# WeijingShi/Point-GNN

Measured on AMD Instinct MI355X. Metric: KITTI-shaped frames/sec (car_auto_T3 inference: graph build + GNN, 20000 pts/frame, mean E1 602k), higher is better.
Workload: dtype f32

## Files before the change

include/pointgnn_hip.h:

```cpp
#ifndef POINTGNN_HIP_H_
#define POINTGNN_HIP_H_

#include <stddef.h>
#include <stdint.h>

#ifdef __cplusplus
extern "C" {
#endif

#define PGNN_E_INVALID (-1)
#define PGNN_E_WORKSPACE (-2)
#define PGNN_E_UNSUPPORTED (-3)
#define PGNN_E_CAPACITY (-4)
#define PGNN_E_COMM (-5)

int pgnn_version(void);
const char *pgnn_last_error(void);
int pgnn_check_device_pointer(const void *device_ptr);

int pgnn_stream_create_cu_mask(int32_t cu_first, int32_t cu_count,
                               int32_t complement, void **stream_out);
int pgnn_stream_destroy(void *stream);

int pgnn_scatter_max_f32(const float *data, int64_t ld_data,
// ... 304 lines not shown
    int32_t edges_sorted, float *out, int64_t ld_out, int32_t *sched_ws,
    int32_t aggregation, void *workspace, size_t workspace_bytes, void *stream);
int pgnn_point_set_pooling_agg_fwd_dyn(
    const float *point_features, int32_t n_feat, const float *point_xyz,
    const int32_t *keypoint_indices, const int32_t *edges, int64_t edges_cap,
    int32_t keypoints_cap, const pgnn_fc_layer *layers_host, int32_t n_layers,
    int32_t edges_sorted, float *out, int64_t ld_out, int32_t *sched_ws,
    const pgnn_dyn_count *n_edges, const pgnn_dyn_count *num_keypoints,
    int32_t aggregation, void *workspace, size_t workspace_bytes, void *stream);

size_t pgnn_packed_fc_bf16x3_bytes(int32_t k_in, int32_t n_out);
int pgnn_pack_fc_bf16x3(const float *w_host, const float *b_host, int32_t k_in,
                        int32_t n_out, void *image_host);
int pgnn_edge_mlp_scatter_max_bf16x3_fwd(
    const float *P, const float *Q, int64_t ld_pq, int32_t width,
    const int32_t *edges, int64_t edges_cap, int32_t vertices_cap,
    const void *image, int32_t n_out, int32_t relu_from, int32_t edges_sorted,
    float *out, int64_t ld_out, const pgnn_dyn_count *n_edges,
    const pgnn_dyn_count *num_vertices, void *stream);

size_t pgnn_packed_fc_f16x2_bytes(int32_t k_in, int32_t n_out);
int pgnn_pack_fc_f16x2(const float *w_host, const float *b_host, int32_t k_in,
                       int32_t n_out, void *image_host);
int pgnn_edge_mlp_scatter_max_f16x2_fwd(
    const float *P, const float *Q, int64_t ld_pq, int32_t width,
    const int32_t *edges, int64_t edges_cap, int32_t vertices_cap,
    const void *image, int32_t n_out, int32_t relu_from, int32_t edges_sorted,
    float *out, int64_t ld_out, int32_t *status, const pgnn_dyn_count *n_edges,
    const pgnn_dyn_count *num_vertices, void *stream);

int pgnn_edge_ws_applies(const pgnn_fc_layer *layers_host, int32_t n_layers,
                         int32_t width, int64_t edges_expected, void *stream,
                         int32_t *applies);
int pgnn_edge_mlp_scatter_max_scaled_fwd(
    const float *P, const float *Q, int64_t ld_pq, int32_t width,
    const int32_t *edges, int64_t edges_cap, int32_t vertices_cap,
    const pgnn_fc_layer *layers_host, int32_t n_layers, int32_t edges_sorted,
    float *out, int64_t ld_out, int32_t *sched_ws, int32_t scale_exp,
    int32_t *status, const pgnn_dyn_count *n_edges,
    const pgnn_dyn_count *num_vertices, void *stream);
int pgnn_debug_pk_sub_clamp(const float *a, const float *b, float *out,
                            int32_t n_pairs, void *stream);

int pgnn_pack_fc_f16x2_acc(const float *w_host, const float *b_host,
                           int32_t k_in, int32_t n_out, void *image_host);
int pgnn_point_set_pooling_f16x2_fwd(
    const float *point_features, int32_t n_feat, const float *point_xyz,
    const int32_t *keypoint_indices, const int32_t *edges, int64_t edges_cap,
    int32_t keypoints_cap, const pgnn_fc_layer *layers, int32_t n_layers,
    const void *last_image, const void *hidden_image, int32_t edges_sorted,
    float *out, int64_t ld_out, int32_t *sched_ws, int32_t *status,
    const pgnn_dyn_count *n_edges, const pgnn_dyn_count *num_keypoints,
    void *stream);

int pgnn_edge_mlp_scatter_max_rows_fwd(const float *P, const float *Q,
                                       int64_t ld_pq, int32_t width,
                                       const int32_t *edges, int64_t n_edges,
                                       int32_t num_vertices,
                                       const pgnn_fc_layer *layer_host,
                                       int32_t edges_sorted, float *out,
                                       int64_t ld_out, float *rows_out,
                                       int64_t ld_rows, float *h1_out,
                                       void *stream);

int pgnn_offset_apply(const float *xyz, const float *delta, int64_t ld_delta,
                      int64_t n_rows, const float *wx, float *xyz_out,
// ... 607 lines not shown
```

point-gnn_amd/_lib.py:

```python
import ctypes
import os

import torch

from . import _header

_HERE = os.path.dirname(os.path.abspath(__file__))
LIB_PATH = os.environ.get("PGNN_LIB") or os.path.join(_HERE, "libpointgnn_hip.so")

c_i32, c_i64, c_vp = ctypes.c_int32, ctypes.c_int64, ctypes.c_void_p

_S, _C = _header.structs(), _header.constants()

FcLayer = _S["pgnn_fc_layer"]
DynCount = _S["pgnn_dyn_count"]
WgradJob = _S["pgnn_wgrad_job"]
MergeJob = _S["pgnn_merge_job"]
FrameArrays = _S["pgnn_frame_arrays"]
TrainFc = _S["pgnn_train_fc"]
TrainStage = _S["pgnn_train_stage"]
TrainModel = _S["pgnn_train_model"]
TrainBatch = _S["pgnn_train_batch"]


class PackJob(ctypes.Structure):
    _fields_ = [("w", c_vp), ("b", c_vp), ("dst", c_vp), ("k_in", c_i32),
                ("n_out", c_i32), ("kind", c_i32), ("first_block", c_i32),
                ("ld", c_i32), ("reserved", c_i32)]


PGNN_MAX_LAYERS = _C["PGNN_MAX_LAYERS"]
MERGE_MAX_LEVELS = _C["PGNN_MERGE_MAX_LEVELS"]
TRAIN_MAX_FC = _C["PGNN_TRAIN_MAX_FC"]
TRAIN_MAX_STAGES = _C["PGNN_TRAIN_MAX_STAGES"]
TRAIN_MAX_CLASSES = _C["PGNN_TRAIN_MAX_CLASSES"]
TRAIN_MAX_LEVELS = _C["PGNN_TRAIN_MAX_LEVELS"]
E_INVALID = _C["PGNN_E_INVALID"]
E_WORKSPACE = _C["PGNN_E_WORKSPACE"]
E_UNSUPPORTED = _C["PGNN_E_UNSUPPORTED"]
AGG_MAX, AGG_SUM, AGG_MEAN = (_C["PGNN_AGG_MAX"], _C["PGNN_AGG_SUM"],
                              _C["PGNN_AGG_MEAN"])
SCHED_WS_INTS = _C["PGNN_SCHED_WS_INTS"]


class PointGnnHipError(RuntimeError):
    pass


_lib = None


def exported_symbols():
    return sorted(_header.functions())


def _build_missing():
    import fcntl
    import shutil
    if not (shutil.which("hipcc") or os.path.exists("/opt/rocm/bin/hipcc")):
        return
    lock = os.path.join(os.path.dirname(LIB_PATH), ".build.lock")
    with open(lock, "w") as f:
        fcntl.flock(f, fcntl.LOCK_EX)
        try:
            if not os.path.exists(LIB_PATH):
                from . import build as _build
                _build.build(verbose=False)
        finally:
            fcntl.flock(f, fcntl.LOCK_UN)


def load():
    global _lib
    if _lib is not None:
        return _lib
# ... 87 lines not shown
```

point-gnn_amd/csrc/core.hip:

```cpp
#include <cmath>
#include <string.h>

#include <mutex>
#include <vector>

#include "pgnn_common.h"

namespace pgnn {

std::string &last_error() {
  static thread_local std::string err;
  return err;
}

namespace {
__global__ void sched_zero_kernel(int32_t *sched) {
  if (threadIdx.x < PGNN_SCHED_WS_INTS) sched[threadIdx.x] = 0;
}
}

int arm_sched(int32_t *sched, hipStream_t stream) {
  if (!sched) return 0;
  static_assert(PGNN_SCHED_WS_INTS <= 64, "one wave zeroes the counters");
  hipLaunchKernelGGL(sched_zero_kernel, dim3(1), dim3(64), 0, stream, sched);
// ... 371 lines not shown

extern "C" size_t pgnn_packed_fc_bf16x3_bytes(int32_t k_in, int32_t n_out) {
  return packed_split_bytes<SplitBf16x3>(k_in, n_out);
}

extern "C" size_t pgnn_packed_fc_f16x2_bytes(int32_t k_in, int32_t n_out) {
  return packed_split_bytes<SplitF16x2>(k_in, n_out);
}

extern "C" int pgnn_pack_fc_bf16x3(const float *w, const float *b, int32_t k_in,
                                   int32_t n_out, void *image) {
  PGNN_GUARD_BEGIN
  PGNN_REQUIRE(w && image && k_in > 0 && n_out > 0, PGNN_E_INVALID,
               "pack_fc_bf16x3: bad argument");
  pack_fc_split<SplitBf16x3>(w, b, k_in, n_out, image, false);
  return 0;
  PGNN_GUARD_END
}

extern "C" int pgnn_pack_fc_f16x2(const float *w, const float *b, int32_t k_in,
                                  int32_t n_out, void *image) {
  PGNN_GUARD_BEGIN
  return pack_fc_f16x2(w, b, k_in, n_out, image, false);
  PGNN_GUARD_END
}

extern "C" int pgnn_pack_fc_f16x2_acc(const float *w, const float *b,
                                      int32_t k_in, int32_t n_out, void *image) {
  PGNN_GUARD_BEGIN
  return pack_fc_f16x2(w, b, k_in, n_out, image, true);
  PGNN_GUARD_END
}

extern "C" int pgnn_pack_fc(const float *w, const float *b, int32_t k_in,
                            int32_t n_out, float *packed) {
  PGNN_GUARD_BEGIN
  PGNN_REQUIRE(w && packed && k_in > 0 && n_out > 0, PGNN_E_INVALID,
               "pack_fc: bad argument");
  const int kq = (k_in + 15) / 16, nt = (n_out + 15) / 16;
  for (int q = 0; q < kq; ++q)
    for (int t = 0; t < nt; ++t)
      for (int lane = 0; lane < 64; ++lane)
        for (int s = 0; s < 4; ++s) {
          const int k = 16 * q + 4 * (lane >> 4) + s;
          const int n = 16 * t + (lane & 15);
          packed[(((size_t)q * nt + t) * 64 + lane) * 4 + s] =
              (k < k_in && n < n_out) ? w[(size_t)k * n_out + n] : 0.0f;
        }
  float *bias = packed + (size_t)kq * nt * 256;
  for (int n = 0; n < nt * 16; ++n) bias[n] = (b && n < n_out) ? b[n] : 0.0f;
  return 0;
  PGNN_GUARD_END
}
```

point-gnn_amd/csrc/edge_ws.h:

```cpp
#pragma once
#include "mlp_engine.h"
#include "ws_partition.h"

namespace pgnn {

#ifndef PGNN_WS_SCHED
#define PGNN_WS_SCHED 2
#endif

constexpr int kWsWaves = 8;
constexpr int kWsSchedInts = 2 + kWsMaxSlices * kWsMaxGroups;
constexpr int kWsStampTiles = 38;
constexpr int kWsStampStride = 8 + 4 * kWsStampTiles;

struct EdgeWsArgs {
  const float *P, *Q;
  int ldv4;
  const int32_t *edges;
  int64_t n_edges;
  const int32_t *n_dev;
  const float *wp;
  int nt;
  int relu_from;
  float *out;
// ... 147 lines not shown
  }
  while (pos < 16) {
    if (cur_has)
      ws_flush<NTG, ARGS, SCALED>(a, bias_lds, t0, lane, cur_d, carry,
                    a.sorted && cur_left_closed &&
                        (!fin || d_after != cur_d),
                    inf);
    if (fin) break;
    const unsigned rest = starts & ~((2u << pos) - 1u);
    const int nextpos = rest ? __builtin_ctz(rest) : 16;
    const bool in_run = n >= pos && n < nextpos;
#pragma unroll
    for (int t = 0; t < NTG; ++t)
#pragma unroll
      for (int r = 0; r < 4; ++r)
        carry[t][r] = in_run ? acc[t][r] : kFloatLowest;
    cur_d = __builtin_amdgcn_readlane(my_d, pos);
    cur_left_closed = true;
    cur_has = true;
    pos = nextpos;
  }
  st.cur_d = cur_d;
  st.left_closed = cur_left_closed;
  st.has = cur_has;
}

}

#include "ws_sum.h"

namespace pgnn {

template <int KQ, int NTG, bool EMIT, bool ROWS = false, class POL = WsMax,
          bool SCALED = false>
__device__ __forceinline__ void edge_ws_body(const EdgeWsArgs &a,
                                             const v4f *__restrict__ wl, int t0,
                                             const float *bias_lds,
                                             int64_t tile_first,
                                             int64_t tile_last, int lane,
                                             long long *tsw, int &stamped,
                                             const int64_t E) {
  static_assert(!SCALED || (!EMIT && !ROWS && !POL::kSum),
                "the scaled form exists for the plain max kernel only");
  if (tile_first >= tile_last) return;
  const int n = lane & 15;
  const int64_t e_first = tile_first * 16;
  const int64_t e_end = tile_last * 16 < E ? tile_last * 16 : E;
  const v4f *__restrict__ P4 = reinterpret_cast<const v4f *>(a.P);
  const v4f *__restrict__ Q4 = reinterpret_cast<const v4f *>(a.Q);
  const int2 *__restrict__ e2 = reinterpret_cast<const int2 *>(a.edges);

  int cur_d = e_first > 0 ? a.edges[2 * (e_first - 1) + 1] : -1;
  int d_after = e_end < E ? a.edges[2 * e_end + 1] : -1;
  cur_d = __builtin_amdgcn_readfirstlane(cur_d);
  d_after = __builtin_amdgcn_readfirstlane(d_after);
  bool cur_left_closed = false, cur_has = false;
  constexpr float kIdentity = POL::kSum ? 0.0f : kFloatLowest;
  v4f carry[NTG];
#pragma unroll
  for (int t = 0; t < NTG; ++t)
    carry[t] = (v4f){kIdentity, kIdentity, kIdentity, kIdentity};

  const float inf = opaque_inf();
  bool nxt_ok = e_first + n < E;
  int2 nxt = e2[nxt_ok ? e_first + n : 0];
  for (int64_t tile = tile_first;; ++tile) {
    const bool fin = tile >= tile_last;
    const int64_t e0 = tile * 16;
    if (a.prio) __builtin_amdgcn_s_setprio(3);
    int lz;
    asm volatile("v_mov_b32 %0, %1" : "=v"(lz) : "v"(lane));
    const int g = lz >> 4;
    int lz1 = lz + 64 * 64, lz2 = lz + 128 * 64;
    asm volatile("" : "+v"(lz1));
    asm volatile("" : "+v"(lz2));
    const v4f *__restrict__ wfrag[3] = {wl + lz, wl + lz1, wl + lz2};
// ... 64 lines not shown
        for (int q = 0; q < KQ; ++q) hrow[4 * q] = in[q];
      }
    }
    __builtin_amdgcn_sched_barrier(0);
    if (tst) {
      const long long c = __builtin_readcyclecounter();
      if (lane == 0) tst[1] = c;
      __builtin_amdgcn_sched_barrier(0);
    }
    __builtin_amdgcn_s_setprio(0);
    {
      v4f w[2][NTG];
#pragma unroll
      for (int t = 0; t < NTG; ++t) {
        acc[t] = (v4f){0.f, 0.f, 0.f, 0.f};
        w[0][t] = wfrag[0][t * 64];
      }
      __builtin_amdgcn_sched_barrier(0);
#pragma unroll
      for (int q = 0; q < KQ; ++q) {
        __builtin_amdgcn_s_waitcnt(0xC07F);
        __builtin_amdgcn_sched_barrier(0);
        if (q + 1 < KQ) {
#pragma unroll
          for (int t = 0; t < NTG; ++t)
#ifdef PGNN_WS_ABL_NO_LDS
            w[(q + 1) & 1][t] = w[q & 1][t];
#else
            w[(q + 1) & 1][t] = wfrag[((q + 1) * NTG + t) >> 6]
                                     [(((q + 1) * NTG + t) & 63) * 64];
#endif
        }
#pragma unroll
        for (int s = 0; s < 4; ++s)
#pragma unroll
          for (int t = 0; t < NTG; ++t)
            acc[t] = __builtin_amdgcn_mfma_f32_16x16x4f32(
                w[q & 1][t][s], in[q][s], acc[t], 0, 0, 0);
#if PGNN_WS_SCHED == 2
#pragma unroll
        for (int t = 0; t < NTG; ++t) {
          __builtin_amdgcn_sched_group_barrier(0x8 , 3, 0);
          if (q + 1 < KQ)
            __builtin_amdgcn_sched_group_barrier(0x100 , 1, 0);
        }
        __builtin_amdgcn_sched_group_barrier(0x8 , NTG, 0);
#else
        if (q + 1 < KQ)
          __builtin_amdgcn_sched_group_barrier(0x100 , NTG, 0);
        __builtin_amdgcn_sched_group_barrier(0x8 , 4 * NTG, 0);
#endif
        __builtin_amdgcn_sched_barrier(0);
      }
    }
    if (tst) {
      const long long c = __builtin_readcyclecounter();
      if (lane == 0) tst[2] = c;
      __builtin_amdgcn_sched_barrier(0);
    }
    if constexpr (EMIT) {
      const int64_t row = e0 + n;
      if (row < E) {
        float *dstp = a.rows_out + row * a.ld_rows + 16 * t0 + 4 * g;
#pragma unroll
        for (int t = 0; t < NTG; ++t) {
          const v4f bb = *reinterpret_cast<const v4f *>(bias_lds + 16 * t + 4 * g);
          v4f y;
#pragma unroll
          for (int r = 0; r < 4; ++r) {
            float x = acc[t][r] + bb[r];
            if (16 * (t0 + t) + 4 * g + r >= a.relu_from) x = x > 0.0f ? x : 0.0f;
            y[r] = x;
          }
          *reinterpret_cast<v4f *>(dstp + 16 * t) = y;
        }
      }
    }
    if (a.prio) __builtin_amdgcn_s_setprio(3);
    const int up = __shfl_up(my_d, 1);
// ... 134 lines not shown
                         __HIP_MEMORY_SCOPE_AGENT);
    }
  }
}

__device__ __forceinline__ void ws_scaled_guard(const EdgeWsArgs &a) {
  if (!a.status) return;
  int nv = a.num_segments;
  if (a.nv_dev) {
    const int d = *a.nv_dev;
    nv = d < nv ? d : nv;
  }
  const v4f *__restrict__ P4 = reinterpret_cast<const v4f *>(a.P);
  const v4f *__restrict__ Q4 = reinterpret_cast<const v4f *>(a.Q);
  float m = 0.0f;
  bool bad = false;
  const int mine = nv > (int)blockIdx.x
                       ? (nv - (int)blockIdx.x + (int)gridDim.x - 1) / (int)gridDim.x
                       : 0;
  for (int it = threadIdx.x; it < mine * a.ldv4; it += 64 * kWsWaves) {
    const int j = it / a.ldv4, c = it - j * a.ldv4;
    const size_t at = ((size_t)blockIdx.x + (size_t)j * gridDim.x) * a.ldv4 + c;
    const v4f p = P4[at], q = Q4[at];
#pragma unroll
    for (int i = 0; i < 4; ++i) {
      m = fmaxf(m, fmaxf(fabsf(p[i]), fabsf(q[i])));
      bad |= !(p[i] == p[i]) || !(q[i] == q[i]);
    }
  }
  if (bad || !(m <= 0.5f)) atomicOr(a.status, 1);
}

template <int KQ, int NTMAX, bool EMIT = false, bool ROWS = false,
          class POL = WsMax, bool SCALED = false>
__global__ __launch_bounds__(64 * kWsWaves) void edge_ws_kernel(EdgeWsArgs a) {
  extern __shared__ __attribute__((aligned(16))) char smem[];
  v4f *wl = reinterpret_cast<v4f *>(smem);
  float *bias_lds = reinterpret_cast<float *>(wl + KQ * NTMAX * 64);
  const int lane = threadIdx.x & 63;
  const int wave = __builtin_amdgcn_readfirstlane(threadIdx.x >> 6);
  const int slice = blockIdx.x % a.xcds;
  const int local = blockIdx.x / a.xcds;
  if constexpr (SCALED) ws_scaled_guard(a);
  const long long rt_entry = a.ts ? (long long)__builtin_amdgcn_s_memrealtime() : 0;
  const int grp = ws_group(a, slice, local, wave);
  const int t0 = a.tile0[grp];
  const int ntg = a.tile0[grp + 1] - t0;
  {
    const v4f *__restrict__ src = reinterpret_cast<const v4f *>(a.wp);
    constexpr int PER = (KQ * NTMAX + kWsWaves - 1) / kWsWaves;
    const int n_frag = KQ * ntg;
    v4f tmp[PER];
#pragma unroll
    for (int i = 0; i < PER; ++i) {
      const int f = wave + i * kWsWaves;
      const int fc = f < n_frag ? f : 0;
      const int q = fc / ntg, t = fc - q * ntg;
      tmp[i] = src[((size_t)q * a.nt + t0 + t) * 64 + lane];
    }
    __builtin_amdgcn_sched_barrier(0);
#pragma unroll
    for (int i = 0; i < PER; ++i) {
      const int f = wave + i * kWsWaves;
      if (f < n_frag) wl[(size_t)f * 64 + lane] = tmp[i];
    }
    if ((int)threadIdx.x < 16 * ntg)
      bias_lds[threadIdx.x] =
          a.wp[(size_t)KQ * a.nt * 256 + 16 * t0 + threadIdx.x];
  }
  __syncthreads();
  const int64_t n_edges = ws_edge_count(a.n_edges, a.n_dev);
  const WsShare s = ws_share(a, grp, slice, local, wave, (n_edges + 15) / 16);
  int64_t span = s.last - s.first;
  const int64_t pool = ws_pool_size(span, a.sched, a.pool_pct, 4, s.nw);
  span -= pool;
  const int64_t pool_first = s.first + span;
  int64_t tile_first = s.first + span * s.wi / s.nw;
  int64_t tile_last = s.first + span * (s.wi + 1) / s.nw;
  long long *tsw = nullptr;
  if (a.ts) {
    tsw = a.ts + ((int64_t)blockIdx.x * kWsWaves + wave) * kWsStampStride;
    if (lane == 0) {
      tsw[0] = __builtin_readcyclecounter();
      tsw[2] = __builtin_amdgcn_s_memrealtime();
      tsw[4] = tile_last - tile_first;
      tsw[5] = ntg + 100 * slice;
      tsw[6] = rt_entry;
    }
  }
  int stamped = 0;
  int32_t *counter = a.sched ? a.sched + 2 + slice * kWsMaxGroups + grp : nullptr;
  for (;;) {
    if (ntg == NTMAX)
      edge_ws_body<KQ, NTMAX, EMIT, ROWS, POL, SCALED>(
          a, wl, t0, bias_lds, tile_first, tile_last, lane, tsw, stamped,
          n_edges);
    else
      edge_ws_body<KQ, NTMAX - 1, EMIT, ROWS, POL, SCALED>(
          a, wl, t0, bias_lds, tile_first, tile_last, lane, tsw, stamped,
          n_edges);
    if (pool == 0) break;
    const int c = ws_pool_claim(counter, a.chunk, lane);
    if (c >= pool) break;
    tile_first = pool_first + c;
    tile_last = tile_first + a.chunk < s.last ? tile_first + a.chunk : s.last;
  }
  if (tsw && lane == 0) {
    tsw[1] = __builtin_readcyclecounter();
    tsw[3] = __builtin_amdgcn_s_memrealtime();
    tsw[7] = stamped;
  }
  if (a.sched && lane == 0) {
    const int total = (int)gridDim.x * kWsWaves;
    const int done = __hip_atomic_fetch_add(&a.sched[1], 1, __ATOMIC_ACQ_REL,
                                            __HIP_MEMORY_SCOPE_AGENT);
    if (done == total - 1) {
      for (int i = 0; i < a.xcds * kWsMaxGroups; ++i)
        __hip_atomic_store(&a.sched[2 + i], 0, __ATOMIC_RELAXED,
                           __HIP_MEMORY_SCOPE_AGENT);
      __hip_atomic_store(&a.sched[1], 0, __ATOMIC_RELEASE,
                         __HIP_MEMORY_SCOPE_AGENT);
    }
  }
}

}
```

point-gnn_amd/csrc/gnn.hip:

```cpp
#include <atomic>

#include "mlp_engine.h"
#include "edge_ws.h"
#include "edge_ws_split.h"
#include "pool_ws.h"
#include "pool_split.h"
#include "pool_ws_f16.h"

namespace pgnn {
int g_mlp_blocks_per_cu = 4;
int g_edge_msub = 0;
int g_pool_msub = 0;
int g_mlp_pool_pct = 12;
int g_ws_xcds = 8;
int g_ws_prio = 1;
int g_f16_pool = 1;
int g_b16_force = 0;
int g_ws_pool_pct = 0;
int g_ws_chunk = 2;
int g_ws_balance = 1;
int g_ws_reserve = 0;
void *g_mlp_ts = nullptr;
int g_mlp_debug = 0;
}
// ... 1170 lines not shown
  Plan p;
  const int rc = make_plan(layers, n_layers, width, p);
  if (rc) return rc;
  *applies = edge_ws_applies(p, edges_expected, ws_cus((hipStream_t)stream_));
  return 0;
  PGNN_GUARD_END
}

extern "C" int pgnn_edge_mlp_scatter_max_scaled_fwd(
    const float *P, const float *Q, int64_t ld_pq, int32_t width,
    const int32_t *edges, int64_t edges_cap, int32_t vertices_cap,
    const pgnn_fc_layer *layers, int32_t n_layers, int32_t edges_sorted,
    float *out, int64_t ld_out, int32_t *sched_ws, int32_t scale_exp,
    int32_t *status, const pgnn_dyn_count *n_edges,
    const pgnn_dyn_count *num_vertices, void *stream_) {
  PGNN_GUARD_BEGIN
  hipStream_t stream = (hipStream_t)stream_;
  PGNN_REQUIRE(edges_cap >= 0 && vertices_cap >= 0 && width > 0,
               PGNN_E_INVALID, "edge_mlp_scaled: bad sizes");
  PGNN_REQUIRE(scale_exp >= 0 && scale_exp <= 24, PGNN_E_INVALID,
               "edge_mlp_scaled: scale_exp outside 0..24");
  PGNN_REQUIRE((n_edges == nullptr) == (num_vertices == nullptr) &&
                   (!n_edges || (n_edges->dev && num_vertices->dev)),
               PGNN_E_INVALID, "edge_mlp_scaled: counts come as a pair");
  const Dyn de = dyn_of(n_edges), dk = dyn_of(num_vertices);
  Plan p;
  int rc = make_plan(layers, n_layers, width, p);
  if (rc) return rc;
  PGNN_REQUIRE(ld_pq == 16 * p.chain.l[0].kq, PGNN_E_INVALID,
               "edge_mlp_scaled: ld_pq must equal the padded width 16*ceil(width/16)");
  PGNN_REQUIRE(ld_out >= 16 * p.chain.l[n_layers - 1].nt, PGNN_E_INVALID,
               "edge_mlp_scaled: ld_out < padded output width");
  const int cus = ws_cus(stream);
  if (edges_cap == 0 || vertices_cap == 0 ||
      !edge_ws_applies(p, expected(de, edges_cap), cus))
    return PGNN_E_UNSUPPORTED;
  PGNN_REQUIRE(out && P && Q && edges, PGNN_E_INVALID,
               "edge_mlp_scaled: null pointer");
  PGNN_REQUIRE(((uintptr_t)P % 16 == 0) && ((uintptr_t)Q % 16 == 0),
               PGNN_E_INVALID, "edge_mlp_scaled: P/Q must be 16-byte aligned");
  if (!(edges_sorted & 2)) {
    rc = fill_lowest_rows(out, ld_out, vertices_cap, dk, stream);
    if (rc) return rc;
  }
  const EdgeArgs ea = {P, Q, ld_pq, edges};
  const SegArgs sa = {out, ld_out, vertices_cap, edges_sorted & 1};
  if (p.chain.l[0].nt == 19)
    return launch_edge_ws_scaled<19, 7>(p.chain.l[0], ea, edges_cap, sa, cus,
                                        sched_ws, stream, de.dev, dk.dev,
                                        scale_exp, status);
  return launch_edge_ws_scaled<16, 8>(p.chain.l[0], ea, edges_cap, sa, cus,
                                      sched_ws, stream, de.dev, dk.dev,
                                      scale_exp, status);
  PGNN_GUARD_END
}

extern "C" int pgnn_edge_mlp_scatter_max_bf16x3_fwd(
    const float *P, const float *Q, int64_t ld_pq, int32_t width,
    const int32_t *edges, int64_t edges_cap, int32_t vertices_cap,
    const void *image, int32_t n_out, int32_t relu_from, int32_t edges_sorted,
    float *out, int64_t ld_out, const pgnn_dyn_count *n_edges,
    const pgnn_dyn_count *num_vertices, void *stream_) {
  PGNN_GUARD_BEGIN
  return edge_split_fwd_impl<Bf16x3>(P, Q, ld_pq, width, edges, edges_cap,
                                     vertices_cap, image, n_out, relu_from,
                                     edges_sorted, out, ld_out, nullptr, n_edges,
                                     num_vertices, (hipStream_t)stream_);
  PGNN_GUARD_END
}

extern "C" int pgnn_edge_mlp_scatter_max_f16x2_fwd(
    const float *P, const float *Q, int64_t ld_pq, int32_t width,
    const int32_t *edges, int64_t edges_cap, int32_t vertices_cap,
    const void *image, int32_t n_out, int32_t relu_from, int32_t edges_sorted,
    float *out, int64_t ld_out, int32_t *status, const pgnn_dyn_count *n_edges,
    const pgnn_dyn_count *num_vertices, void *stream_) {
  PGNN_GUARD_BEGIN
  return edge_split_fwd_impl<F16x2>(P, Q, ld_pq, width, edges, edges_cap,
                                    vertices_cap, image, n_out, relu_from,
// ... 1230 lines not shown
```

point-gnn_amd/csrc/ws_launch.h:

```cpp
#pragma once
#include "ws_partition.h"

namespace {
using namespace pgnn;

inline int ws_cus(int cus) {
  return (g_ws_reserve > 0 && cus - g_ws_reserve >= 64) ? cus - g_ws_reserve : cus;
}
inline int ws_cus(hipStream_t stream) { return ws_cus(stream_cu_count(stream)); }

inline int ws_slices(int cus) { return ws_slice_count(cus, g_ws_xcds); }
inline bool ws_feasible(int nt, int ntmax, int cus) {
  return pgnn::ws_feasible(nt, ntmax, cus, ws_slices(cus));
}

inline int ws_partition_rc(int why) {
  PGNN_REQUIRE(why != kWsTooFewCus, PGNN_E_UNSUPPORTED,
               "edge_ws: too few CUs for the column groups");
  PGNN_REQUIRE(why == kWsOk, PGNN_E_UNSUPPORTED,
               "edge_ws: column tiles do not group");
  return 0;
}

template <int KQ, int NTMAX>
// ... 4 lines not shown
  a = {};
  const int rc = ws_partition_rc(ws_partition(a, L.nt, NTMAX, cus, ws_slices(cus)));
  if (rc) return rc;
  a.n_dev = n_dev;
  a.rows_out = rows_out;
  a.ld_rows = ld_rows;
  a.h1_out = h1_out;
  a.P = ea.P;
  a.Q = ea.Q;
  a.ldv4 = (int)(ea.ldpq >> 2);
  a.edges = ea.edges;
  a.n_edges = n_edges;
  a.wp = L.wp;
  a.nt = L.nt;
  a.relu_from = L.relu_from;
  a.out = sa.out;
  a.ldo = sa.ldo;
  a.num_segments = sa.num_segments;
  a.sorted = sa.sorted;
  a.prio = g_ws_prio;
  a.ts = (long long *)g_mlp_ts;
  a.sched = (g_ws_pool_pct > 0 && a.xcds <= kWsMaxSlices) ? sched : nullptr;
  a.pool_pct = g_ws_pool_pct;
  a.chunk = g_ws_chunk;
  if (g_ws_balance >= 2) {
    double cost[kWsMaxGroups];
    for (int g = 0; g < a.groups; ++g)
      cost[g] = 128.0 * KQ * (a.tile0[g + 1] - a.tile0[g]) + 1900.0;
    ws_balance(a, cus, cost, a.sched != nullptr);
  }
  return 0;
}

template <int KQ, int NTMAX, bool ROWS, class POL = WsMax, bool SCALED = false>
int run_edge_ws(const EdgeWsArgs &a, int cus, hipStream_t stream) {
  static_assert(!POL::kSum || !ROWS, "the sum kernels read no ready rows");
  static_assert(!SCALED || (!POL::kSum && !ROWS), "scaled: the plain max kernel only");
  PGNN_HIP((hipError_t)arm_sched(a.sched, stream));
  const size_t lds = (size_t)KQ * NTMAX * 1024 + 16 * NTMAX * sizeof(float);
  auto kern = edge_ws_kernel<KQ, NTMAX, false, ROWS, POL, SCALED>;
  if constexpr (!ROWS && !POL::kSum && !SCALED) {
    if (a.rows_out) kern = edge_ws_kernel<KQ, NTMAX, true>;
  }
  return launch_lds(kern, dim3((unsigned)(cus / a.xcds * a.xcds)),
                    dim3(64 * kWsWaves), lds, stream, a);
}

template <int KQ, int NTMAX, class POL = WsMax>
int launch_edge_ws(const LayerDev &L, const EdgeArgs &ea, int64_t n_edges,
                   const SegArgs &sa, int cus, int32_t *sched,
                   hipStream_t stream, float *rows_out = nullptr,
                   int64_t ld_rows = 0, float *h1_out = nullptr,
                   const int32_t *n_dev = nullptr) {
  EdgeWsArgs a;
  const int rc = plan_edge_ws<KQ, NTMAX>(a, L, ea, n_edges, sa, cus, sched,
                                         rows_out, ld_rows, h1_out, n_dev);
  return rc ? rc : run_edge_ws<KQ, NTMAX, false, POL>(a, cus, stream);
}

template <int KQ, int NTMAX>
int launch_edge_ws_scaled(const LayerDev &L, const EdgeArgs &ea, int64_t n_edges,
                          const SegArgs &sa, int cus, int32_t *sched,
                          hipStream_t stream, const int32_t *n_dev,
                          const int32_t *nv_dev, int scale_exp, int32_t *status) {
  EdgeWsArgs a;
  const int rc = plan_edge_ws<KQ, NTMAX>(a, L, ea, n_edges, sa, cus, sched,
                                         nullptr, 0, nullptr, n_dev);
  if (rc) return rc;
  a.nv_dev = nv_dev;
  a.unscale = (float)((int64_t)1 << scale_exp);
  a.status = status;
  return run_edge_ws<KQ, NTMAX, false, WsMax, true>(a, cus, stream);
}

template <class POL = WsMax>
bool edge_ws_applies(const Plan &p, int64_t n_edges, int cus) {
  if (g_mlp_debug & 2048) return false;
  const LayerDev &L = p.chain.l[0];
  if (p.chain.n != 1 || L.kq != L.nt || (L.nt != 19 && L.nt != 16)) return false;
  if (cus < 64 || cus % 8 != 0) return false;
  if (!ws_feasible(L.nt, L.nt == 19 ? 7 : 8, cus)) return false;
  if ((size_t)L.kq * (L.nt == 19 ? 7 : 8) * 1024 + 16 * 8 * sizeof(float) >
      device_max_lds())
    return false;
  if (g_mlp_debug & 4096) return true;
  return n_edges >= (int64_t)16 * 2 * kWsWaves * cus;
}

template <class POL = WsMax>
bool pool_ws_applies(const Plan &p, int64_t n_edges, int cus) {
  if (g_mlp_debug & (8192 | 1024)) return false;
  const ChainDev &c = p.chain;
  if (c.n != 4 || c.l[0].kq != 1 || c.l[0].nt != 2 || c.l[1].nt != 4 ||
      c.l[2].nt != 8 || c.l[3].kq != 8 || c.l[3].nt != 19)
    return false;
  if (cus < 8) return false;
  if ((size_t)8 * 19 * 1024 + 16 * 19 * sizeof(float) > device_max_lds())
    return false;
  if (g_mlp_debug & 16384) return true;
  return n_edges >= (int64_t)16 * 2 * kWsWaves * cus;
}

PoolWsArgs pool_ws_args(const Plan &p, const PoolArgs &pa, int64_t n_edges,
                        const int32_t *n_dev, int num_segments) {
  PoolWsArgs a = {};
  a.feat = pa.feat;
  a.nfeat = pa.nfeat;
  a.xyz = pa.xyz;
  a.kp = pa.kp;
  a.edges = pa.edges;
  a.n_edges = n_edges;
  a.n_dev = n_dev;
  a.l0 = p.chain.l[0];
  a.l1 = p.chain.l[1];
  a.l2 = p.chain.l[2];
  a.wp = p.chain.l[3].wp;
  a.kq = p.chain.l[3].kq;
  a.nt = p.chain.l[3].nt;
  a.relu_from = p.chain.l[3].relu_from;
// ... 183 lines not shown
```

point-gnn_amd/gnn.py:

```python
import contextlib
import ctypes
import threading
from functools import partial

import numpy as np
import torch

from . import _lib
from .weights import mlp_names

__all__ = ["PointSetPooling", "GraphNetAutoCenter", "ClassAwarePredictor",
           "fuse_vertex_stages",
           "multi_layer_neural_network_fn", "multi_layer_fc_fn",
           "graph_scatter_max_fn", "graph_scatter_sum_fn",
           "graph_scatter_mean_fn", "ParamStore", "parameters",
           "variable_scope", "padded_width"]


def padded_width(n):
    return (int(n) + 15) // 16 * 16


class ParamStore(object):

    def __init__(self, params, device=None):
        self.params = {k: np.asarray(v) for k, v in params.items()}
        self.device = device
        self._cache = {}
        self._edge_arith = 'f32'
        self.edge_scaled = False
        self.inference = True

    @property
    def edge_arith(self):
        return self._edge_arith

    @edge_arith.setter
    def edge_arith(self, value):
        if value not in EDGE_ARITHS:
            raise ValueError("edge_arith must be one of %r, not %r"
                             % (EDGE_ARITHS, value))
        self._edge_arith = value

    def range_status(self):
        if getattr(self, '_range_status', None) is None:
            self._range_status = torch.zeros(1, dtype=torch.int32,
                                             device=self._dev())
        return self._range_status

    def edge_range_ok(self):
        st = getattr(self, '_range_status', None)
        if st is None:
            return True
        ok = int(st.item()) == 0
        if not ok:
            st.zero_()
        return ok

    def edge_scale_exp(self, scope):
        scales = self.__dict__.setdefault('_edge_scale', {})
        pend = self.__dict__.setdefault('_edge_scale_pending', {})
        if scope not in scales and scope in pend and \
                not torch.cuda.is_current_stream_capturing():
# ... 66 lines not shown
    def _dev(self):
        if self.device is None:
            if not torch.cuda.is_available():
                raise _lib.PointGnnHipError(
                    "pointgnn_amd needs a GPU: there is no CPU fallback")
            self.device = torch.device("cuda", torch.cuda.current_device())
        return self.device

    def has(self, name):
        return name + '/weights' in self.params

    def fc(self, name):
        w = self.params[name + '/weights']
        if name + '/biases' in self.params:
            return (w.astype(np.float32),
                    self.params[name + '/biases'].astype(np.float32))
        bn = name + '/BatchNorm/'
        if bn + 'moving_mean' not in self.params:
            raise KeyError("%s: neither biases nor BatchNorm statistics"
                           % name)
        mean = self.params[bn + 'moving_mean'].astype(np.float64)
        var = self.params[bn + 'moving_variance'].astype(np.float64)
        s = 1.0 / np.sqrt(var + BATCH_NORM_EPSILON)
        if bn + 'gamma' in self.params:
            s = s * self.params[bn + 'gamma'].astype(np.float64)
        beta = self.params[bn + 'beta'].astype(np.float64) \
            if bn + 'beta' in self.params else 0.0
        return ((w.astype(np.float64) * s).astype(np.float32),
                (beta - mean * s).astype(np.float32))

    def mlp(self, scope, n_layers):
        return [self.fc(n) for n in mlp_names(scope, n_layers)]

    def pack(self, w, b):
        lib = _lib.load()
        w = np.ascontiguousarray(w, dtype=np.float32)
        b = np.ascontiguousarray(b, dtype=np.float32)
        k_in, n_out = w.shape
        host = np.empty(lib.pgnn_packed_fc_floats(k_in, n_out), np.float32)
        _lib.check(lib.pgnn_pack_fc(w.ctypes.data, b.ctypes.data, k_in, n_out,
                                    host.ctypes.data), "pgnn_pack_fc")
        return torch.from_numpy(host).to(self._dev())

    def cached(self, key, builder):
        if key not in self._cache:
            self._cache[key] = builder()
        return self._cache[key]

    def invalidate(self):
        self._cache.clear()


class Chain(object):

    def __init__(self, store, layers):
        self.buffers = []
        self.array = (_lib.FcLayer * len(layers))()
        self.n = len(layers)
        for i, (w, b, relu_from) in enumerate(layers):
            buf = store.pack(w, b)
            self.buffers.append(buf)
            self.array[i].packed = buf.data_ptr()
            self.array[i].k_in = int(w.shape[0])
            self.array[i].n_out = int(w.shape[1])
            self.array[i].relu_from = int(relu_from)
        self.k_in = int(layers[0][0].shape[0])
        self.n_out = int(layers[-1][0].shape[1])


class _State(threading.local):

    def __init__(self):
        self.store = None
        self.scope = []
        self.fuse = False
        self.pending = None
        self.taken = None


_state = _State()


@contextlib.contextmanager
def parameters(store):
    prev = _state.store
    _state.store = store
    try:
        yield store
    finally:
        _state.store = prev


@contextlib.contextmanager
# ... 403 lines not shown
                "pgnn_point_set_pooling_workspace_bytes")
        if done:
            pass
        elif ws_bytes.value:
            work = torch.empty(ws_bytes.value // 4, dtype=torch.float32,
                               device=xyz.device)
            _lib.check(lib.pgnn_point_set_pooling_fwd_ws(
                *args, cnt_e.arg() if cnt_e is not None else None,
                cnt_k.arg() if cnt_k is not None else None, _lib.ptr(work),
                ws_bytes.value, _lib.stream_ptr()),
                "pgnn_point_set_pooling_fwd_ws")
        elif cnt_k is None and cnt_e is None:
            _lib.check(lib.pgnn_point_set_pooling_fwd(
                *args, _lib.stream_ptr()), "pgnn_point_set_pooling_fwd")
        else:
            _lib.check(lib.pgnn_point_set_pooling_fwd_dyn(
                *args, cnt_e.arg(), cnt_k.arg(), _lib.stream_ptr()),
                "pgnn_point_set_pooling_fwd_dyn")
        if AGGREGATE_TAP is not None:
            AGGREGATE_TAP.append(agg)
        with variable_scope('combined_features'):
            out_chain = _relu_chain(store, _scope(),
                                    list(output_MLP_depth_list), False)
        return _finish_rows(out_chain, agg, point_chain.n_out, count=cnt_k)


EDGE_INPUT_TAP = None

EDGE_ARITHS = ('f32', 'bf16x3', 'f16x2')

EDGE_SCALE_HEADROOM = 0.125
EDGE_SCALE_ROWS, EDGE_SCALE_SLOTS = 64, 16


def edge_scale_exp_for(max_abs):
    k = 0
    while k < 24 and not max_abs * 2.0 ** -k <= EDGE_SCALE_HEADROOM:
        k += 1
    return k


class GraphNetAutoCenter(object):

    def __init__(self, edge_feature_fn=multi_layer_neural_network_fn,
                 aggregation_fn=graph_scatter_max_fn,
                 update_fn=multi_layer_neural_network_fn,
                 auto_offset_fn=multi_layer_neural_network_fn):
        self._aggregation = _aggregation_code(aggregation_fn)
        self._edge_feature_fn = edge_feature_fn
        self._aggregation_fn = aggregation_fn
        self._update_fn = update_fn
        self._auto_offset_fn = auto_offset_fn

    def apply_regular(self, input_vertex_features, input_vertex_coordinates,
                      NOT_USED, edges, edge_MLP_depth_list=None,
                      edge_MLP_normalization_type='fused_BN_center',
                      edge_MLP_activation_type='ReLU',
                      update_MLP_depth_list=None,
                      update_MLP_normalization_type='fused_BN_center',
                      update_MLP_activation_type='ReLU', auto_offset=False,
                      auto_offset_MLP_depth_list=None,
                      auto_offset_MLP_normalization_type='fused_BN_center',
                      auto_offset_MLP_feature_activation_type='ReLU'):
        _check_kinds(edge_MLP_activation_type, edge_MLP_normalization_type)
        _check_kinds(update_MLP_activation_type, update_MLP_normalization_type)
        pend = _take_pending(input_vertex_features)
# ... 20 lines not shown
            fcs = store.mlp(edge_scope, len(edge_widths))
            w1, b1 = fcs[0]
            c = w1.shape[0] - 3
            p_chain = Chain(store, [(w1, b1, w1.shape[1])])
            wq = padded_width(w1.shape[1])
            wx = np.zeros((3, wq), np.float32)
            wx[:, :w1.shape[1]] = w1[c:c + 3]
            wx_dev = torch.from_numpy(wx).to(store._dev())
            if len(fcs) > 1:
                rest = Chain(store, [(w, b, 0) for (w, b) in fcs[1:]])
            else:
                rest = None
            return c, p_chain, wx_dev, rest
        c, p_chain, wx_dev, rest = store.cached(
            ('edge', edge_scope, tuple(edge_widths)), build_edge)
        if rest is None:
            raise NotImplementedError("edge MLP needs at least two layers")
        assert h.shape[1] >= c, "vertex features narrower than edge MLP input"

        scale_k, calibrate = None, False
        if store.edge_scaled and store.inference and rest.n == 1 and \
                store.edge_arith == 'f32' and \
                self._aggregation == _lib.AGG_MAX:
            n_exp = int(e.shape[0])
            if cnt_e is not None and 0 < cnt_e.hint < n_exp:
                n_exp = cnt_e.hint
            applies = ctypes.c_int32(0)
            _lib.check(lib.pgnn_edge_ws_applies(
                rest.array, rest.n, int(rest.k_in), n_exp, st,
                ctypes.byref(applies)), "pgnn_edge_ws_applies")
            if applies.value:
                scale_k = store.edge_scale_exp(edge_scope)
                calibrate = scale_k is None and cnt_k is None
        if scale_k is not None:
            def build_scaled():
                w1, b1 = store.mlp(edge_scope, len(edge_widths))[0]
                s = np.float32(2.0 ** -scale_k)
                wx = np.zeros((3, padded_width(w1.shape[1])), np.float32)
                wx[:, :w1.shape[1]] = w1[c:c + 3] * s
                made = (Chain(store, [(w1 * s, b1 * s, w1.shape[1])]),
                        torch.from_numpy(wx).to(store._dev()))
                torch.cuda.current_stream().synchronize()
                return made
            p_chain, wx_dev = store.cached(
                ('edge_scaled', edge_scope, tuple(edge_widths), scale_k),
                build_scaled)

        off_chain = None
        if auto_offset:
            _check_kinds(auto_offset_MLP_feature_activation_type,
                         auto_offset_MLP_normalization_type)
            off_chain = _relu_chain(store, scope,
                                    list(auto_offset_MLP_depth_list), True)
            assert off_chain.k_in == c, "offset MLP input must be the features"
        wq = int(wx_dev.shape[1])
        q = torch.empty((k, wq), dtype=torch.float32, device=h.device)
        p = torch.empty((k, wq), dtype=torch.float32, device=h.device)
        agg = torch.empty((k, padded_width(rest.n_out)), dtype=torch.float32,
                          device=h.device)
        pre_args = (_lib.ptr(h), h.stride(0), c, _lib.ptr(x),
                    off_chain.array if off_chain is not None else None,
                    off_chain.n if off_chain is not None else 0, p_chain.array,
                    _lib.ptr(wx_dev), k, _lib.ptr(p), _lib.ptr(q), wq,
                    _lib.ptr(agg), agg.stride(0))
        if pend is not None:
            res = pend.residual
            front = (_lib.ptr(pend.x), pend.x.stride(0), pend.nx,
                     pend.chain.array, pend.chain.n, _lib.ptr(res),
                     res.stride(0) if res is not None else 0, _lib.ptr(h),
                     h.stride(0))
            if cnt_k is None:
                rc = lib.pgnn_vertex_update_pre_edge_fwd(
                    *(front + pre_args[2:]), st)
            else:
                rc = lib.pgnn_vertex_update_pre_edge_fwd_dyn(
                    *(front + pre_args[2:]), cnt_k.arg(), st)
            if rc == _lib.E_UNSUPPORTED:
                _flush_pending()
                pend = None
            else:
                _lib.check(rc, "pgnn_vertex_update_pre_edge_fwd")
                _tail_launched()
        if pend is not None:
            pass
        elif cnt_k is None:
            _lib.check(lib.pgnn_vertex_pre_edge_fwd(*pre_args, st),
                       "pgnn_vertex_pre_edge_fwd")
        else:
            _lib.check(lib.pgnn_vertex_pre_edge_fwd_dyn(
                *pre_args, cnt_k.arg(), st), "pgnn_vertex_pre_edge_fwd_dyn")
        if calibrate:
            store.note_edge_range(edge_scope, p, q)
        if EDGE_INPUT_TAP is not None:
            EDGE_INPUT_TAP.append((p, q))
        edge_args = (_lib.ptr(p), _lib.ptr(q), wq, int(rest.k_in), _lib.ptr(e),
                     int(e.shape[0]), k, rest.array, rest.n,
                     _edges_sorted_flag(edges) | 2, _lib.ptr(agg),
                     agg.stride(0), _lib.ptr(_lib.sched_ws(h.device)))
        done = False
        if self._aggregation != _lib.AGG_MAX:
            _aggregate(lib, "edge_mlp_scatter_agg",
                       (rest.array, rest.n, int(rest.k_in)), edge_args,
                       int(e.shape[0]), k, cnt_e, cnt_k, self._aggregation,
                       h.device)
            done = True
        elif store.edge_arith != 'f32' and rest.n == 1:
            done = self._edge_split(lib, store, edge_scope, edge_widths, p, q,
                                    wq, rest, e, k, edges, agg, cnt_e, cnt_k,
                                    st)
        elif scale_k is not None:
            _lib.check(lib.pgnn_edge_mlp_scatter_max_scaled_fwd(
                *edge_args, scale_k, store.edge_scale_status(edge_scope),
                cnt_e.arg() if cnt_e is not None else None,
                cnt_k.arg() if cnt_k is not None else None, st),
                "pgnn_edge_mlp_scatter_max_scaled_fwd")
            done = True
        if done:
            pass
        elif cnt_k is None:
            _lib.check(lib.pgnn_edge_mlp_scatter_max_fwd(*edge_args, st),
                       "pgnn_edge_mlp_scatter_max_fwd")
        else:
            _lib.check(lib.pgnn_edge_mlp_scatter_max_fwd_dyn(
                *edge_args, cnt_e.arg(), cnt_k.arg(), st),
                "pgnn_edge_mlp_scatter_max_fwd_dyn")
        if AGGREGATE_TAP is not None:
            AGGREGATE_TAP.append(agg)
        upd_chain = _relu_chain(store, scope + '/combined_features',
                                list(update_MLP_depth_list), True)
        assert upd_chain.n_out == c, "update MLP must preserve the width"
        if h.shape[1] < padded_width(c):
            hp = torch.zeros((k, padded_width(c)), dtype=torch.float32,
                             device=h.device)
            hp[:, :h.shape[1]] = h
            h = hp
        return _finish_rows(upd_chain, agg, rest.n_out, residual=h,
                            count=cnt_k)


    @staticmethod
    def _edge_split(lib, store, edge_scope, edge_widths, p, q, wq, rest, e, k,
                    edges, agg, cnt_e, cnt_k, st):
        arith = store.edge_arith

        def build():
# ... 188 lines not shown
```

point-gnn_amd/models.py:

```python
from functools import partial

import numpy as np
import torch

from . import _lib, gnn
from .weights import init_params

__all__ = ["MultiLayerFastLocalGraphModelV2", "get_model", "cls_loss_kind",
           "loss_top_k", "top_k_selection"]


def cls_loss_kind(cls_loss_type, cls_loss_kwargs=None):
    kw = cls_loss_kwargs or {}
    if cls_loss_type == 'softmax':
        return 0, 0.0, 0.0
    if cls_loss_type == 'focal_softmax':
        return 1, 0.0, float(kw.get('gamma', 2))
    if cls_loss_type == 'focal_sigmoid':
        return 2, float(kw.get('alpha', 0.5)), float(kw.get('gamma', 2))
    if cls_loss_type == 'top_k_softmax':
        return 0, 0.0, 0.0
    raise ValueError("cls_loss_type %r (models.py:210-211 knows softmax, "
                     "top_k_softmax, focal_sigmoid, focal_softmax)"
                     % (cls_loss_type,))
# ... 89 lines not shown
                               num_layer=3)),
        }
        assert mode in ['train', 'eval', 'test'], 'Unsupported mode'
        self._mode = mode
        self._store = None
        self._edge_arith = 'f32'

    @property
    def edge_arith(self):
        return self._edge_arith

    @edge_arith.setter
    def edge_arith(self, value):
        if value not in gnn.EDGE_ARITHS:
            raise ValueError("edge_arith must be one of %r, not %r"
                             % (gnn.EDGE_ARITHS, value))
        self._edge_arith = value
        if self._store is not None:
            self._store.edge_arith = value

    def edge_range_ok(self):
        return self._store is None or self._store.edge_range_ok()

    @property
    def edge_scaled(self):
        return getattr(self, '_edge_scaled', True)

    @edge_scaled.setter
    def edge_scaled(self, value):
        self._edge_scaled = bool(value)
        if self._store is not None:
            self._store.edge_scaled = self._edge_scaled

    def edge_scale_begin_pass(self):
        return 0 if self._store is None else \
            self._store.edge_scale_begin_pass()

    def edge_scale_ok(self, rows=None):
        return self._store is None or self._store.edge_scale_ok(rows)

    def edge_scale_flags(self):
        return None if self._store is None else self._store.edge_scale_flags()

    def edge_scale_tripped(self, host, count=True):
        return self._store.edge_scale_tripped(host, count)

    def edge_scale_discard(self, row):
        if self._store is not None:
            self._store.edge_scale_discard(row)

    def edge_scale_exps(self):
        if self._store is None:
            return {}
        return dict(self._store.__dict__.get('_edge_scale', {}))

    def load_state_dict(self, params, device=None):
        self._store = gnn.ParamStore(params, device)
        self._store.edge_arith = self._edge_arith
        self._store.edge_scaled = self.edge_scaled
        return self

    def init_weights(self, config, seed=0, **kw):
        return self.load_state_dict(init_params(config, seed=seed, **kw))

    def state_dict(self):
        return dict(self._store.params)

    def predict(self, t_initial_vertex_features, t_vertex_coord_list,
                t_keypoint_indices_list, t_edges_list, is_training):
        if self._store is None:
            raise RuntimeError("call load_state_dict()/init_weights() first")
        if is_training:
            for cfg in self._layer_configs:
                for key, val in (cfg.get('kwargs') or {}).items():
                    if key.endswith('normalization_type') and \
                            val in gnn.FOLDED_NORMALIZATIONS:
                        raise NotImplementedError(
                            "%s: %s = %r with is_training=True (batch "
                            "statistics) has no device path" % (
                                cfg['scope'], key, val))
        was_np = not isinstance(t_initial_vertex_features, torch.Tensor)
        if was_np:
            dev = self._store._dev()

            def up(a, dt):
                return torch.from_numpy(np.ascontiguousarray(
                    np.asarray(a), dtype=dt)).to(dev)
            t_initial_vertex_features = up(t_initial_vertex_features,
                                           np.float32)
            t_vertex_coord_list = [up(c, np.float32)
                                   for c in t_vertex_coord_list]
            t_keypoint_indices_list = [
# ... 171 lines not shown
```

Baseline: 328.5.

## Reorder K=300 edge MLP inputs to skip the padded final MFMA step

Adds a permutation of the 300-wide input features so the 4 padding columns in the last 16-wide K group all land in a single MFMA k-step. The scaled edge kernel, instantiated with a K300 flag, then runs only 3 of the 4 MFMA steps for the last K group. Both the first-layer output columns and the second layer's input rows are packed in the permuted order, so results are unchanged. It removes about 1/76 of the first-layer MFMA work, adds another kernel instantiation and more packing code, and is on by default.

```diff
diff --git a/include/pointgnn_hip.h b/include/pointgnn_hip.h
--- a/include/pointgnn_hip.h
+++ b/include/pointgnn_hip.h
@@ -360,6 +360,10 @@
 int pgnn_edge_ws_applies(const pgnn_fc_layer *layers_host, int32_t n_layers,
                          int32_t width, int64_t edges_expected, void *stream,
                          int32_t *applies);
+#define PGNN_EDGE_K300_ORDER 4
+int32_t pgnn_k300_source(int32_t position);
+int pgnn_pack_fc_k300(const float *w_host, const float *b_host, int32_t k_in,
+                      int32_t n_out, float *packed_host);
 int pgnn_edge_mlp_scatter_max_scaled_fwd(
     const float *P, const float *Q, int64_t ld_pq, int32_t width,
     const int32_t *edges, int64_t edges_cap, int32_t vertices_cap,
diff --git a/point-gnn_amd/_lib.py b/point-gnn_amd/_lib.py
--- a/point-gnn_amd/_lib.py
+++ b/point-gnn_amd/_lib.py
@@ -41,6 +41,7 @@
 AGG_MAX, AGG_SUM, AGG_MEAN = (_C["PGNN_AGG_MAX"], _C["PGNN_AGG_SUM"],
                               _C["PGNN_AGG_MEAN"])
 SCHED_WS_INTS = _C["PGNN_SCHED_WS_INTS"]
+EDGE_K300_ORDER = _C["PGNN_EDGE_K300_ORDER"]
 
 
 class PointGnnHipError(RuntimeError):
diff --git a/point-gnn_amd/csrc/core.hip b/point-gnn_amd/csrc/core.hip
--- a/point-gnn_amd/csrc/core.hip
+++ b/point-gnn_amd/csrc/core.hip
@@ -427,23 +427,49 @@
   PGNN_GUARD_END
 }
 
-extern "C" int pgnn_pack_fc(const float *w, const float *b, int32_t k_in,
-                            int32_t n_out, float *packed) {
-  PGNN_GUARD_BEGIN
-  PGNN_REQUIRE(w && packed && k_in > 0 && n_out > 0, PGNN_E_INVALID,
-               "pack_fc: bad argument");
+namespace {
+template <class SRC>
+void pack_fc_rows(const float *w, const float *b, int32_t k_in, int32_t n_out,
+                  float *packed, SRC src) {
   const int kq = (k_in + 15) / 16, nt = (n_out + 15) / 16;
   for (int q = 0; q < kq; ++q)
     for (int t = 0; t < nt; ++t)
       for (int lane = 0; lane < 64; ++lane)
         for (int s = 0; s < 4; ++s) {
-          const int k = 16 * q + 4 * (lane >> 4) + s;
+          const int k = src(16 * q + 4 * (lane >> 4) + s);
           const int n = 16 * t + (lane & 15);
           packed[(((size_t)q * nt + t) * 64 + lane) * 4 + s] =
               (k < k_in && n < n_out) ? w[(size_t)k * n_out + n] : 0.0f;
         }
   float *bias = packed + (size_t)kq * nt * 256;
   for (int n = 0; n < nt * 16; ++n) bias[n] = (b && n < n_out) ? b[n] : 0.0f;
-  return 0;
-  PGNN_GUARD_END
-}
+}
+}
+
+extern "C" int pgnn_pack_fc(const float *w, const float *b, int32_t k_in,
+                            int32_t n_out, float *packed) {
+  PGNN_GUARD_BEGIN
+  PGNN_REQUIRE(w && packed && k_in > 0 && n_out > 0, PGNN_E_INVALID,
+               "pack_fc: bad argument");
+  pack_fc_rows(w, b, k_in, n_out, packed, [](int k) { return k; });
+  return 0;
+  PGNN_GUARD_END
+}
+
+extern "C" int32_t pgnn_k300_source(int32_t position) {
+  if (position < 288 || position >= 304) return position;
+  const int g = (position - 288) >> 2, s = (position - 288) & 3, j = 4 * s + g;
+  return j < 12 ? 288 + 4 * (j % 3) + j / 3 : 300 + g;
+}
+
+extern "C" int pgnn_pack_fc_k300(const float *w, const float *b, int32_t k_in,
+                                 int32_t n_out, float *packed) {
+  PGNN_GUARD_BEGIN
+  PGNN_REQUIRE(w && packed && n_out > 0, PGNN_E_INVALID,
+               "pack_fc_k300: bad argument");
+  PGNN_REQUIRE(k_in == 300, PGNN_E_UNSUPPORTED,
+               "pack_fc_k300: the order exists for 300 input features only");
+  pack_fc_rows(w, b, k_in, n_out, packed, pgnn_k300_source);
+  return 0;
+  PGNN_GUARD_END
+}
diff --git a/point-gnn_amd/csrc/edge_ws.h b/point-gnn_amd/csrc/edge_ws.h
--- a/point-gnn_amd/csrc/edge_ws.h
+++ b/point-gnn_amd/csrc/edge_ws.h
@@ -203,7 +203,7 @@
 namespace pgnn {
 
 template <int KQ, int NTG, bool EMIT, bool ROWS = false, class POL = WsMax,
-          bool SCALED = false>
+          bool SCALED = false, bool K300 = false>
 __device__ __forceinline__ void edge_ws_body(const EdgeWsArgs &a,
                                              const v4f *__restrict__ wl, int t0,
                                              const float *bias_lds,
@@ -213,6 +213,8 @@
                                              const int64_t E) {
   static_assert(!SCALED || (!EMIT && !ROWS && !POL::kSum),
                 "the scaled form exists for the plain max kernel only");
+  static_assert(!K300 || (SCALED && KQ == 19),
+                "the K = 300 form exists for the scaled kernel of 19 K groups");
   if (tile_first >= tile_last) return;
   const int n = lane & 15;
   const int64_t e_first = tile_first * 16;
@@ -343,7 +345,7 @@
 #endif
         }
 #pragma unroll
-        for (int s = 0; s < 4; ++s)
+        for (int s = 0; s < (K300 && q == KQ - 1 ? 3 : 4); ++s)
 #pragma unroll
           for (int t = 0; t < NTG; ++t)
             acc[t] = __builtin_amdgcn_mfma_f32_16x16x4f32(
@@ -355,7 +357,8 @@
           if (q + 1 < KQ)
             __builtin_amdgcn_sched_group_barrier(0x100 , 1, 0);
         }
-        __builtin_amdgcn_sched_group_barrier(0x8 , NTG, 0);
+        if (!(K300 && q == KQ - 1))
+          __builtin_amdgcn_sched_group_barrier(0x8 , NTG, 0);
 #else
         if (q + 1 < KQ)
           __builtin_amdgcn_sched_group_barrier(0x100 , NTG, 0);
@@ -556,7 +559,7 @@
 }
 
 template <int KQ, int NTMAX, bool EMIT = false, bool ROWS = false,
-          class POL = WsMax, bool SCALED = false>
+          class POL = WsMax, bool SCALED = false, bool K300 = false>
 __global__ __launch_bounds__(64 * kWsWaves) void edge_ws_kernel(EdgeWsArgs a) {
   extern __shared__ __attribute__((aligned(16))) char smem[];
   v4f *wl = reinterpret_cast<v4f *>(smem);
@@ -616,11 +619,11 @@
   int32_t *counter = a.sched ? a.sched + 2 + slice * kWsMaxGroups + grp : nullptr;
   for (;;) {
     if (ntg == NTMAX)
-      edge_ws_body<KQ, NTMAX, EMIT, ROWS, POL, SCALED>(
+      edge_ws_body<KQ, NTMAX, EMIT, ROWS, POL, SCALED, K300>(
           a, wl, t0, bias_lds, tile_first, tile_last, lane, tsw, stamped,
           n_edges);
     else
-      edge_ws_body<KQ, NTMAX - 1, EMIT, ROWS, POL, SCALED>(
+      edge_ws_body<KQ, NTMAX - 1, EMIT, ROWS, POL, SCALED, K300>(
           a, wl, t0, bias_lds, tile_first, tile_last, lane, tsw, stamped,
           n_edges);
     if (pool == 0) break;
diff --git a/point-gnn_amd/csrc/gnn.hip b/point-gnn_amd/csrc/gnn.hip
--- a/point-gnn_amd/csrc/gnn.hip
+++ b/point-gnn_amd/csrc/gnn.hip
@@ -1226,8 +1226,10 @@
   PGNN_REQUIRE(ld_out >= 16 * p.chain.l[n_layers - 1].nt, PGNN_E_INVALID,
                "edge_mlp_scaled: ld_out < padded output width");
   const int cus = ws_cus(stream);
+  const bool k300 = (edges_sorted & PGNN_EDGE_K300_ORDER) != 0;
   if (edges_cap == 0 || vertices_cap == 0 ||
-      !edge_ws_applies(p, expected(de, edges_cap), cus))
+      !edge_ws_applies(p, expected(de, edges_cap), cus) ||
+      (k300 && !edge_k300_applies(p, layers, width)))
     return PGNN_E_UNSUPPORTED;
   PGNN_REQUIRE(out && P && Q && edges, PGNN_E_INVALID,
                "edge_mlp_scaled: null pointer");
@@ -1239,6 +1241,10 @@
   }
   const EdgeArgs ea = {P, Q, ld_pq, edges};
   const SegArgs sa = {out, ld_out, vertices_cap, edges_sorted & 1};
+  if (k300)
+    return launch_edge_ws_scaled<19, 7, true>(p.chain.l[0], ea, edges_cap, sa,
+                                              cus, sched_ws, stream, de.dev,
+                                              dk.dev, scale_exp, status);
   if (p.chain.l[0].nt == 19)
     return launch_edge_ws_scaled<19, 7>(p.chain.l[0], ea, edges_cap, sa, cus,
                                         sched_ws, stream, de.dev, dk.dev,
diff --git a/point-gnn_amd/csrc/ws_launch.h b/point-gnn_amd/csrc/ws_launch.h
--- a/point-gnn_amd/csrc/ws_launch.h
+++ b/point-gnn_amd/csrc/ws_launch.h
@@ -60,13 +60,14 @@
   return 0;
 }
 
-template <int KQ, int NTMAX, bool ROWS, class POL = WsMax, bool SCALED = false>
+template <int KQ, int NTMAX, bool ROWS, class POL = WsMax, bool SCALED = false,
+          bool K300 = false>
 int run_edge_ws(const EdgeWsArgs &a, int cus, hipStream_t stream) {
   static_assert(!POL::kSum || !ROWS, "the sum kernels read no ready rows");
   static_assert(!SCALED || (!POL::kSum && !ROWS), "scaled: the plain max kernel only");
   PGNN_HIP((hipError_t)arm_sched(a.sched, stream));
   const size_t lds = (size_t)KQ * NTMAX * 1024 + 16 * NTMAX * sizeof(float);
-  auto kern = edge_ws_kernel<KQ, NTMAX, false, ROWS, POL, SCALED>;
+  auto kern = edge_ws_kernel<KQ, NTMAX, false, ROWS, POL, SCALED, K300>;
   if constexpr (!ROWS && !POL::kSum && !SCALED) {
     if (a.rows_out) kern = edge_ws_kernel<KQ, NTMAX, true>;
   }
@@ -86,7 +87,7 @@
   return rc ? rc : run_edge_ws<KQ, NTMAX, false, POL>(a, cus, stream);
 }
 
-template <int KQ, int NTMAX>
+template <int KQ, int NTMAX, bool K300 = false>
 int launch_edge_ws_scaled(const LayerDev &L, const EdgeArgs &ea, int64_t n_edges,
                           const SegArgs &sa, int cus, int32_t *sched,
                           hipStream_t stream, const int32_t *n_dev,
@@ -98,7 +99,7 @@
   a.nv_dev = nv_dev;
   a.unscale = (float)((int64_t)1 << scale_exp);
   a.status = status;
-  return run_edge_ws<KQ, NTMAX, false, WsMax, true>(a, cus, stream);
+  return run_edge_ws<KQ, NTMAX, false, WsMax, true, K300>(a, cus, stream);
 }
 
 template <class POL = WsMax>
@@ -113,6 +114,12 @@
     return false;
   if (g_mlp_debug & 4096) return true;
   return n_edges >= (int64_t)16 * 2 * kWsWaves * cus;
+}
+
+inline bool edge_k300_applies(const Plan &p, const pgnn_fc_layer *layers,
+                              int width) {
+  return p.chain.n == 1 && p.chain.l[0].kq == 19 && p.chain.l[0].nt == 19 &&
+         layers[0].k_in == 300 && width == 300;
 }
 
 template <class POL = WsMax>
diff --git a/point-gnn_amd/gnn.py b/point-gnn_amd/gnn.py
--- a/point-gnn_amd/gnn.py
+++ b/point-gnn_amd/gnn.py
@@ -29,6 +29,7 @@
         self._cache = {}
         self._edge_arith = 'f32'
         self.edge_scaled = False
+        self.edge_k300 = EDGE_K300
         self.inference = True
 
     @property
@@ -161,14 +162,15 @@
     def mlp(self, scope, n_layers):
         return [self.fc(n) for n in mlp_names(scope, n_layers)]
 
-    def pack(self, w, b):
+    def pack(self, w, b, k300=False):
         lib = _lib.load()
         w = np.ascontiguousarray(w, dtype=np.float32)
         b = np.ascontiguousarray(b, dtype=np.float32)
         k_in, n_out = w.shape
         host = np.empty(lib.pgnn_packed_fc_floats(k_in, n_out), np.float32)
-        _lib.check(lib.pgnn_pack_fc(w.ctypes.data, b.ctypes.data, k_in, n_out,
-                                    host.ctypes.data), "pgnn_pack_fc")
+        name = "pgnn_pack_fc_k300" if k300 else "pgnn_pack_fc"
+        _lib.check(getattr(lib, name)(w.ctypes.data, b.ctypes.data, k_in,
+                                      n_out, host.ctypes.data), name)
         return torch.from_numpy(host).to(self._dev())
 
     def cached(self, key, builder):
@@ -182,12 +184,12 @@
 
 class Chain(object):
 
-    def __init__(self, store, layers):
+    def __init__(self, store, layers, k300=False):
         self.buffers = []
         self.array = (_lib.FcLayer * len(layers))()
         self.n = len(layers)
         for i, (w, b, relu_from) in enumerate(layers):
-            buf = store.pack(w, b)
+            buf = store.pack(w, b, k300)
             self.buffers.append(buf)
             self.array[i].packed = buf.data_ptr()
             self.array[i].k_in = int(w.shape[0])
@@ -657,6 +659,22 @@
 EDGE_SCALE_HEADROOM = 0.125
 EDGE_SCALE_ROWS, EDGE_SCALE_SLOTS = 64, 16
 
+EDGE_K300 = True
+
+
+def edge_k300_order(n=304):
+    lib = _lib.load()
+    return np.array([lib.pgnn_k300_source(p) for p in range(n)], np.int64)
+
+
+def edge_k300_columns(a, width=304):
+    a = np.asarray(a, np.float32)
+    src = edge_k300_order(width)
+    out = np.zeros(a.shape[:-1] + (width,), np.float32)
+    real = src < a.shape[-1]
+    out[..., real] = a[..., src[real]]
+    return out
+
 
 def edge_scale_exp_for(max_abs):
     k = 0
@@ -743,19 +761,28 @@
             if applies.value:
                 scale_k = store.edge_scale_exp(edge_scope)
                 calibrate = scale_k is None and cnt_k is None
+        k300 = scale_k is not None and store.edge_k300 and \
+            EDGE_INPUT_TAP is None and rest.k_in == 300
+        rest_k = rest
         if scale_k is not None:
             def build_scaled():
-                w1, b1 = store.mlp(edge_scope, len(edge_widths))[0]
+                fcs = store.mlp(edge_scope, len(edge_widths))
+                w1, b1 = fcs[0]
                 s = np.float32(2.0 ** -scale_k)
+                if k300:
+                    w1, b1 = edge_k300_columns(w1), edge_k300_columns(b1)
                 wx = np.zeros((3, padded_width(w1.shape[1])), np.float32)
                 wx[:, :w1.shape[1]] = w1[c:c + 3] * s
                 made = (Chain(store, [(w1 * s, b1 * s, w1.shape[1])]),
-                        torch.from_numpy(wx).to(store._dev()))
+                        torch.from_numpy(wx).to(store._dev()),
+                        Chain(store, [fcs[1] + (0,)], k300=True)
+                        if k300 else None)
                 torch.cuda.current_stream().synchronize()
                 return made
-            p_chain, wx_dev = store.cached(
-                ('edge_scaled', edge_scope, tuple(edge_widths), scale_k),
+            p_chain, wx_dev, rest_k = store.cached(
+                ('edge_scaled', edge_scope, tuple(edge_widths), scale_k, k300),
                 build_scaled)
+            rest_k = rest_k or rest
 
         off_chain = None
         if auto_offset:
@@ -820,8 +847,11 @@
                                     wq, rest, e, k, edges, agg, cnt_e, cnt_k,
                                     st)
         elif scale_k is not None:
+            flags = edge_args[9] | (_lib.EDGE_K300_ORDER if k300 else 0)
             _lib.check(lib.pgnn_edge_mlp_scatter_max_scaled_fwd(
-                *edge_args, scale_k, store.edge_scale_status(edge_scope),
+                *(edge_args[:7] + (rest_k.array, rest_k.n, flags) +
+                  edge_args[10:]),
+                scale_k, store.edge_scale_status(edge_scope),
                 cnt_e.arg() if cnt_e is not None else None,
                 cnt_k.arg() if cnt_k is not None else None, st),
                 "pgnn_edge_mlp_scatter_max_scaled_fwd")
diff --git a/point-gnn_amd/models.py b/point-gnn_amd/models.py
--- a/point-gnn_amd/models.py
+++ b/point-gnn_amd/models.py
@@ -145,6 +145,16 @@
         if self._store is not None:
             self._store.edge_scaled = self._edge_scaled
 
+    @property
+    def edge_k300(self):
+        return getattr(self, '_edge_k300', gnn.EDGE_K300)
+
+    @edge_k300.setter
+    def edge_k300(self, value):
+        self._edge_k300 = bool(value)
+        if self._store is not None:
+            self._store.edge_k300 = self._edge_k300
+
     def edge_scale_begin_pass(self):
         return 0 if self._store is None else \
             self._store.edge_scale_begin_pass()
@@ -171,6 +181,7 @@
         self._store = gnn.ParamStore(params, device)
         self._store.edge_arith = self._edge_arith
         self._store.edge_scaled = self.edge_scaled
+        self._store.edge_k300 = self.edge_k300
         return self
 
     def init_weights(self, config, seed=0, **kw):
```

Result: faster. 332.0 (median of 6 runs) (+1.1%).
